# tlk00/BitMagic

Hardware: AMD Instinct MI355X
Metric: Gbits/s + % HBM roofline, 256-way fused AND+COUNT on 1B-bit vectors (higher is better)
Workload: dtype u64; 1 GPU; aggregator pipeline combine_and_sub counts-only: 256-way AND+COUNT, 256 x 1000000000-bit vectors in total, data set A (common 10% OR noise 10%: no early exit); vectors=256, bits_per_vector=1000000000, density_q16=6554, blocks_per_vector=15259, blocks_per_rank=15259, hbm_resident_bytes=32279432448

## Files before the change

### bitmagic_amd/csrc/bmx.hip

```cpp
#include "bmx_internal.h"
#ifdef BMX_DIAG
#include "bmx_diag.h"
#endif
#include "bmx_kernels2.h"
#include "bmx_kernels3.h"
#include "bmx_kernels4.h"
#include "bmx_kernels5.h"
#include "bmx_kernels6.h"
#include "bmx_kernels7.h"
#include "bmx_kernels8.h"
#include "bmx_kernels9.h"
#include "bmx_kernels10.h"
#include "bmx_kernels11.h"
#include "bmx_kernels12.h"
#include "bmx_kernels13.h"
#include "bmx_kernels14.h"

#include <algorithm>
#include <atomic>
#include <chrono>
#include <cstdio>
#include <cstdlib>
#include <cstring>
#include <new>
// ... 616 lines not shown
    }
    size_t need = (bytes + 63u) & ~(size_t)63u;
    if (ctx->stage_off + need > STAGE_BYTES) { HIPCHK(hipEventSynchronize(ctx->ev_stage)); ctx->stage_off = 0; }
    char* s = ctx->h_stage + ctx->stage_off;
    memcpy(s, src, bytes);
    ctx->stage_off += need;
    HIPCHK(hipMemcpyAsync(dst, s, bytes, hipMemcpyHostToDevice, ctx->stream));
    HIPCHK(hipEventRecord(ctx->ev_stage, ctx->stream));
    return BMX_OK;
}

static int coll_members_upload(bmx_ctx* ctx, const std::vector<u32>& ma, const std::vector<u32>& ms, DevBuf& d_buf, const u32** d_midx, const CollGroup** d_groups)
{
    const size_t nm = ma.size() + ms.size(), goff = (nm * 4 + 15) & ~(size_t)15;
    std::vector<u8> h(goff + sizeof(CollGroup));
    if (!ma.empty()) memcpy(h.data(), ma.data(), ma.size() * 4);
    if (!ms.empty()) memcpy(h.data() + ma.size() * 4, ms.data(), ms.size() * 4);
    const CollGroup g{0u, (u32)ma.size(), (u32)ma.size(), (u32)ms.size()};
    memcpy(h.data() + goff, &g, sizeof(g));
    int rc;
    if ((rc = dmalloc(ctx, &d_buf.p, h.size())) || (rc = h2d_staged(ctx, d_buf.p, h.data(), h.size()))) { d_buf.reset(); return rc; }
    *d_midx = (const u32*)d_buf.p; *d_groups = (const CollGroup*)((const char*)d_buf.p + goff);
    return BMX_OK;
}

static bool use_split(const bmx_ctx* ctx, const bmx_pipeline* p, u64 nitems)
{
    if (ctx->pipe_split == 0 || !nitems) return false;
    if (ctx->pipe_split == 1) return nitems <= 65535u * 16u;
    return nitems <= 384u && (u64)p->n_ops >= 24ull * p->ngroups;
}
#define SPLIT_WAVES 8

typedef void (*pipe_bits_fn)(const u64*, const u32*, const u32*, u32, u32, u32, u32, int, u64*);

static u32 pipe_window_cap(u32 wg)
{
    u32 wpb = wg / 64u;
    u32 per_cu = wpb >= 7u ? 1u : 12u / wpb;
    return 256u * per_cu * wpb;
}
static void pipe_plan(const bmx_ctx* ctx, u64 nitems, u32 ngroups, u32& rows, u32& wg, u32& unroll, u32& window)
{
    rows = (u32)ctx->pipe_rows;
    if (!rows) rows = nitems >= 1400u ? 8u : nitems >= 700u ? 4u : nitems >= 350u ? 2u : 1u;
    unroll = ctx->pipe_unroll ? (u32)ctx->pipe_unroll : ((rows >= 4u || !ctx->pipe_nt) ? 4u : 8u);
    u64 n = nitems * (8u / rows);
    wg = (u32)ctx->pipe_wg;
    if (!wg) {
        wg = 256u;
        if (rows == 8u) {
            static const u32 cand[3] = {640u, 768u, 512u};
            double best = -1.0;
            for (u32 c : cand) {
                u64 cap = pipe_window_cap(c), nwin = (n + cap - 1) / cap, per = (n + nwin - 1) / nwin;
                double fill = (double)per / (double)cap;
                if (fill > best + 0.02) { best = fill; wg = c; }
            }
        }
    }
    if (!ctx->pipe_nt && !ctx->pipe_wg && rows == 8u && wg > 512u) wg = 512u;
    if (ctx->pipe_window < 0 || (ctx->pipe_window == 0 && ngroups > 4u)) window = 0u;
    else if (ctx->pipe_window > 0) window = (u32)ctx->pipe_window;
    else window = (u32)std::max<u64>(pipe_window_cap(wg) / ((u64)ngroups * (8u / rows)), 1u);
}

template <int ROWS>
static pipe_bits_fn pipe_bits_rows(u32 unroll, bool nt, u32 wg)
// ... 21 lines not shown
            if (unroll == 4) return B2(4, true, 384);
            if constexpr (ROWS <= 4) { if (unroll == 8) return B2(8, true, 384); }
            if constexpr (ROWS <= 2) { if (unroll == 16) return B2(16, true, 384); }
        }
        if (nt && wg == 512 && unroll == 4) return B2(4, true, 512);
    }
#endif
#undef B2
    return nullptr;
}
static pipe_bits_fn pipe_bits_kernel(u32 rows, u32 unroll, bool nt, u32 wg)
{
    switch (rows) {
    case 8: return pipe_bits_rows<8>(unroll, nt, wg);
    case 4: return pipe_bits_rows<4>(unroll, nt, wg);
    case 2: return pipe_bits_rows<2>(unroll, nt, wg);
    case 1: return pipe_bits_rows<1>(unroll, nt, wg);
    default: return nullptr;
    }
}

static int ctx_set_tuning(bmx_ctx* ctx, const char* key, int value)
{
    ARGCHK(ctx && key);
    std::string k(key);
    if (k == "pipe_unroll") { ARGCHK(value == 0 || value == 1 || value == 2 || value == 4 || value == 8 || value == 16); ctx->pipe_unroll = value; }
    else if (k == "pipe_rows") { ARGCHK(value == 0 || value == 8 || value == 4 || value == 2 || value == 1); ctx->pipe_rows = value; }
    else if (k == "pipe_nt") ctx->pipe_nt = value != 0;
    else if (k == "pipe_lds") { ARGCHK(value >= 0 && value <= 160 * 1024); ctx->pipe_lds = value; }
    else if (k == "pipe_slots") { ARGCHK(value == 8 || value == 16); ctx->pipe_slots = value; }
    else if (k == "pipe_staged") { ARGCHK(value >= -1 && value <= 1); ctx->pipe_staged = value; }
    else if (k == "pipe_split") { ARGCHK(value >= -1 && value <= 1); ctx->pipe_split = value; }
    else if (k == "pipe_window") { ARGCHK(value >= -1); ctx->pipe_window = value; }
    else if (k == "or_tile") { ARGCHK(value >= 0 && value <= 3); ctx->or_tile = value; }
    else if (k == "or_rows") { ARGCHK(value >= -1 && value <= 1); ctx->or_rows = value; }
    else if (k == "or_depth") { ARGCHK(value == 4 || value == 8); ctx->or_depth = value; }
    else if (k == "direct_cols") { ARGCHK(value >= 0); ctx->direct_cols = value; }
    else if (k == "pair_stream") { ARGCHK(value == -1 || value == 0 || value == 2 || value == 4 || value == 8); ctx->pair_stream = value; }
    else if (k == "pair_wgs") { ARGCHK(value >= 1 && value <= 8); ctx->pair_wgs = value; }
    else if (k == "range_halves") { ARGCHK(value == 0 || value == 1); ctx->range_halves = value; }
    else if (k == "gap_count") { ARGCHK(value >= -1 && value <= 1); ctx->gap_count = value; }
    else if (k == "agg_shape") { ARGCHK(value == 0 || value == 1); ctx->agg_shape = value; }
    else if (k == "and_rows") { ARGCHK(value >= -1 && value <= 1); ctx->and_rows = value; }
    else if (k == "and_rows_wg") { ARGCHK(value == 128 || value == 256 || value == 512); ctx->and_rows_wg = value; }
    else if (k == "and_rows_depth") { ARGCHK(value == 2 || value == 3 || value == 4 || value == 8); ctx->and_rows_depth = value; }
    else if (k == "and_rows_nt") ctx->and_rows_nt = value != 0;
    else if (k == "and_rows_ipw") { ARGCHK(value >= 0 && value <= 64); ctx->and_rows_ipw = value; }
    else if (k == "ff_window") { ARGCHK(value >= -1); ctx->ff_window = value; }
    else if (k == "or_window") { ARGCHK(value >= -9); ctx->or_window = value; }
    else if (k == "gap_pack") { ARGCHK(value >= -1 && value <= 1); ctx->gap_pack = value; }
    else if (k == "coll_members") { ARGCHK(value >= -1 && value <= 1); ctx->coll_members = value; ++ctx->coll_gen; }
    else if (k == "coll_shape") { ARGCHK(value >= 0 && value <= 5); ctx->coll_shape = value; }
    else if (k == "op2_nt") { ARGCHK(value >= 0 && value <= 3); ctx->op2_nt = value; }
    else if (k == "op2_loop") { ARGCHK(value >= -1 && value <= 8); ctx->op2_loop = value; }
    else if (k == "op2_wgs") { ARGCHK(value >= 1 && value <= 8); ctx->op2_wgs = value; }
    else if (k == "pair_nt") { ARGCHK(value >= 0 && value <= 1); ctx->pair_nt = value; }
    else if (k == "pair_loop") { ARGCHK(value >= -1 && value <= 5); ctx->pair_loop = value; }
    else if (k == "eq_big_shape") { ARGCHK(value >= 0 && value <= 2); ctx->eq_big_shape = value; }
    else if (k == "eq_big") { ARGCHK(value >= -1 && value <= 1); ctx->eq_big = value; }
    else if (k == "coll_split") { ARGCHK(value == 0 || value == 1); ctx->coll_split = value; }
    else if (k == "coll_build") { ARGCHK(value >= -1 && value <= 1); ctx->coll_build = value; }
    else if (k == "coll_window") { ARGCHK(value >= 0); ctx->coll_window = value; }
    else if (k == "rs_select_lines") { ARGCHK(value >= 0 && value <= 2); ctx->rs_select_lines = value; }
    else if (k == "rs_sdir_shift") { ARGCHK(value == 0 || (value >= 6 && value <= 20)); ctx->rs_sdir_shift = value; }
    else if (k == "rs_lines") { ARGCHK(value >= 0 && value <= 2); ctx->rs_lines = value; }
    else if (k == "rs_sorted_hint") { ARGCHK(value == 0 || value == 1); ctx->rs_sorted_hint = value; }
// ... 112 lines not shown
    HIPCHK(hipGetDeviceCount(&n));
    if (device < 0 || device >= n) { g_last_error = "device index out of range"; return BMX_ERR_RANGE; }
    HIPCHK(hipSetDevice(device));
    Owned<bmx_ctx> ctx(new bmx_ctx());
    ctx->device = device;
    if (stream) ctx->stream = (hipStream_t)stream;
    else { HIPCHK(hipStreamCreateWithFlags(&ctx->stream, hipStreamNonBlocking)); ctx->own_stream = true; }
    HIPCHK(hipEventCreate(&ctx->ev0));
    HIPCHK(hipEventCreate(&ctx->ev1));
    HIPCHK(hipMalloc((void**)&ctx->d_small, 64 * sizeof(u64)));
    HIPCHK(hipHostMalloc((void**)&ctx->h_small, 64 * sizeof(u64)));
    HIPCHK(hipHostMalloc((void**)&ctx->h_stage, STAGE_BYTES));
    HIPCHK(hipEventCreateWithFlags(&ctx->ev_stage, hipEventDisableTiming));
    HIPCHK(hipMalloc((void**)&ctx->d_slots, COUNT_SLOTS * COUNT_SLOT_STRIDE * sizeof(u64)));
    HIPCHK(hipMemsetAsync(ctx->d_slots, 0, COUNT_SLOTS * COUNT_SLOT_STRIDE * sizeof(u64), ctx->stream));
    HIPCHK(hipMalloc((void**)&ctx->d_zero, 256));
    HIPCHK(hipMemsetAsync(ctx->d_zero, 0, 256, ctx->stream));
    HIPCHK(hipMalloc((void**)&ctx->d_done, FOLD_DONE_WORDS * 4));
    HIPCHK(hipMemsetAsync(ctx->d_done, 0, FOLD_DONE_WORDS * 4, ctx->stream));
    HIPCHK(hipMalloc((void**)&ctx->d_slots2, COUNT_SLOTS * COUNT_SLOT_STRIDE * sizeof(u64)));
    HIPCHK(hipMemsetAsync(ctx->d_slots2, 0, COUNT_SLOTS * COUNT_SLOT_STRIDE * sizeof(u64), ctx->stream));
    HIPCHK(hipMalloc((void**)&ctx->d_done2, FOLD_DONE_WORDS * 4));
    HIPCHK(hipMemsetAsync(ctx->d_done2, 0, FOLD_DONE_WORDS * 4, ctx->stream));
    HIPCHK(hipHostMalloc((void**)&ctx->h_pend, PEND_SLOTS * 8 * sizeof(u64)));
    HIPCHK(hipMalloc((void**)&ctx->d_cursor, 64));
    HIPCHK(hipMemsetAsync(ctx->d_cursor, 0, 64, ctx->stream));
    { int v = 0; if (hipDeviceGetAttribute(&v, hipDeviceAttributeMaxSharedMemoryPerBlock, device) == hipSuccess && v > 0) ctx->max_lds_bytes = (uint32_t)v; else (void)hipGetLastError(); }
    { size_t fr = 0, tot = 0; if (hipMemGetInfo(&fr, &tot) == hipSuccess && fr) ctx->pack_cap = (uint64_t)fr / 4; else (void)hipGetLastError(); }
    if (const char* e = getenv("BMX_DEBUG_REDZONE")) ctx->redzone = atoi(e) != 0;
    if (const char* e = getenv("BMX_PACK_MAX_MB")) { long long mb = atoll(e); if (mb >= 0) ctx->pack_cap = (uint64_t)mb << 20; }
    if (const char* e = getenv("BMX_POOL_MAX_MB")) { long long mb = atoll(e); if (mb >= 0) ctx->pool_cap = (uint64_t)mb << 20; }
    static const char* const env_keys[][2] = {
        {"BMX_PIPE_UNROLL", "pipe_unroll"}, {"BMX_PIPE_ROWS", "pipe_rows"}, {"BMX_PIPE_NT", "pipe_nt"},
        {"BMX_PIPE_WG", "pipe_wg"}, {"BMX_PIPE_WINDOW", "pipe_window"}, {"BMX_PIPE_SPLIT", "pipe_split"}, {"BMX_OR_TILE", "or_tile"}, {"BMX_OR_ROWS", "or_rows"}, {"BMX_OR_DEPTH", "or_depth"}, {"BMX_OR_WINDOW", "or_window"}, {"BMX_DIRECT_COLS", "direct_cols"}, {"BMX_FF_WINDOW", "ff_window"}, {"BMX_GAP_COUNT", "gap_count"}, {"BMX_AND_ROWS", "and_rows"}, {"BMX_AGG_SHAPE", "agg_shape"}, {"BMX_AND_ROWS_WG", "and_rows_wg"}, {"BMX_AND_ROWS_DEPTH", "and_rows_depth"}, {"BMX_AND_ROWS_NT", "and_rows_nt"}, {"BMX_AND_ROWS_IPW", "and_rows_ipw"}, {"BMX_RANGE_HALVES", "range_halves"}, {"BMX_PAIR_STREAM", "pair_stream"}, {"BMX_PAIR_WGS", "pair_wgs"}, {"BMX_RS_LANES", "rs_lanes"}, {"BMX_RS_SELECT_TOP", "rs_select_top"}, {"BMX_RS_SELECT_SEL", "rs_select_sel"}, {"BMX_RS_LINES", "rs_lines"}, {"BMX_RS_SELECT_LINES", "rs_select_lines"}, {"BMX_RS_SDIR_SHIFT", "rs_sdir_shift"}, {"BMX_COLL_SHAPE", "coll_shape"}, {"BMX_COLL_WINDOW", "coll_window"}, {"BMX_COLL_SPLIT", "coll_split"}, {"BMX_COLL_BUILD", "coll_build"}, {"BMX_EQ_BIG", "eq_big"}, {"BMX_PAIR_LOOP", "pair_loop"}, {"BMX_PAIR_NT", "pair_nt"}, {"BMX_EQ_BIG_SHAPE", "eq_big_shape"}, {"BMX_OP2_WGS", "op2_wgs"}, {"BMX_OP2_LOOP", "op2_loop"}, {"BMX_OP2_NT", "op2_nt"}, {"BMX_GAP_PACK", "gap_pack"}, {"BMX_COLL_MEMBERS", "coll_members"}, {"BMX_XCD_SWIZZLE", "xcd_swizzle"}};
    for (auto& kv : env_keys)
        if (const char* e = getenv(kv[0])) (void)ctx_set_tuning(ctx.get(), kv[1], atoi(e));
    g_last_error.clear();
    *out = ctx.release();
    return BMX_OK;
ABI_END }

int bmx_ctx_destroy(bmx_ctx* ctx) { ABI_TRY if (ctx) ctx_release(ctx); return BMX_OK; ABI_END }

int bmx_ctx_set_tuning(bmx_ctx* ctx, const char* key, int value) { ABI_TRY return ctx_set_tuning(ctx, key, value); ABI_END }

int bmx_probe_stream_rw(bmx_ctx* ctx, uint64_t bytes, int sets, int wgs_per_cu, int iters, float* ms_per_pass)
{ ABI_TRY
    ARGCHK(ctx && ms_per_pass && bytes >= 8192 && sets >= 1 && sets <= 8 && wgs_per_cu >= 1 && wgs_per_cu <= 8 && iters >= 1);
    int rc = set_dev(ctx); if (rc) return rc;
    const u64 nblk = bytes / 8192;
    if (nblk > 0x7FFFFFFFull) { g_last_error = "probe buffer too large"; return BMX_ERR_RANGE; }
    void* buf = nullptr;
    HIPCHK(hipMalloc(&buf, (size_t)nblk * 8192 * 3 * sets));
    hipError_t e = hipMemsetAsync(buf, 0x5A, (size_t)nblk * 8192 * 3 * sets, ctx->stream);
    const u32 waves = 4u, total = 256u * waves * (u32)wgs_per_cu;
    const u32 per_wave = (u32)((nblk + total - 1u) / total);
    const u32 grid = (u32)(((nblk + per_wave - 1u) / per_wave + waves - 1u) / waves);
    for (int it = -2; it < iters && e == hipSuccess; ++it) {
        if (it == 0) e = hipEventRecord(ctx->ev0, ctx->stream);
        uint4* base = (uint4*)buf + (size_t)((it + 2) % sets) * nblk * 512u * 3u;
        hipLaunchKernelGGL(HIP_KERNEL_NAME(k_probe_rw<4>), dim3(grid), dim3(256), 0, ctx->stream, (const uint4*)base, (const uint4*)(base + nblk * 512u),
                           base + 2u * nblk * 512u, (u32)nblk, per_wave);
    }
    if (e == hipSuccess) e = hipEventRecord(ctx->ev1, ctx->stream);
    if (e == hipSuccess) e = hipEventSynchronize(ctx->ev1);
    float ms = 0;
    if (e == hipSuccess) e = hipEventElapsedTime(&ms, ctx->ev0, ctx->ev1);
// ... 1150 lines not shown
                               (const u64* const*)p->d_udesc, (const u32*)p->d_unblk, p->nplanes, gv ? gv->gmask : (const u32*)p->d_gmask, gv ? gv->gskip : (const u32*)p->d_gskip, \
                               ngroups, nb_from, nb_to - nb_from, ctx->xcd_swz, (u64*)d_counts); } while (0)
            if (ctx->pipe_slots == 8) LAUNCH_STG(8); else LAUNCH_STG(16);
#undef LAUNCH_STG
            KCHK();
            return BMX_OK;
        }
    }
    if (use_split(ctx, p, nitems64)) {
        size_t lds = (size_t)SPLIT_WAVES * 8192;
        auto fn = k_pipe_split<2, SPLIT_WAVES>;
        HIPCHK(hipFuncSetAttribute(reinterpret_cast<const void*>(fn), hipFuncAttributeMaxDynamicSharedMemorySize, (int)lds));
        hipLaunchKernelGGL(fn, dim3((u32)nitems64), dim3(SPLIT_WAVES * 64), lds, ctx->stream,
                           (const u64*)p->d_dmat, row_off, and_n, sub_n, p->col_stride, ngroups, nb_from, nb_to, 0, (u64*)d_counts,
                           0, (uint4*)nullptr, (u64*)nullptr, (BlockStat*)nullptr);
        KCHK();
        return BMX_OK;
    }
    if (!p->has_gap) {
        u32 rows, wg, unroll, window;
        pipe_plan(ctx, nitems64, ngroups, rows, wg, unroll, window);
        u32 parts = 8u / rows;
        if (nitems64 * parts > 0xFFFFFFF0ull) { g_last_error = "too many work items in one run"; return BMX_ERR_RANGE; }
        pipe_bits_fn fn = pipe_bits_kernel(rows, unroll, ctx->pipe_nt != 0, wg);
        if (!fn) { g_last_error = "this (pipe_rows, pipe_unroll, pipe_nt, pipe_wg) shape is not compiled into the library"; return BMX_ERR_BADARG; }
        u32 wpb = wg / 64u;
        u32 ncols = nb_to - nb_from;
        u32 nwin = window ? (ncols + window - 1u) / window : 1u;
        u32 per = (ncols + nwin - 1u) / nwin;
        for (u32 c0 = 0; c0 < ncols; c0 += per) {
            u32 cols = std::min(per, ncols - c0);
            u32 nitems = cols * ngroups * parts, grid = (nitems + wpb - 1) / wpb;
            hipLaunchKernelGGL(fn, dim3(grid), dim3(wg), (size_t)ctx->pipe_lds, ctx->stream,
                               (const u64*)p->d_dmat, row_off, and_n, p->col_stride, ngroups, nb_from + c0, nitems, ctx->xcd_swz, (u64*)d_counts);
            KCHK();
        }
        return BMX_OK;
    }
    if (nitems64 > 0xFFFFFFF0ull) { g_last_error = "too many (column, group) items in one run"; return BMX_ERR_RANGE; }
    if (use_and_rows(ctx, p)) {
        const u32 ipw = ctx->and_rows_ipw > 0 ? (u32)ctx->and_rows_ipw : 1u;
        hipLaunchKernelGGL(and_rows_kernel<AR_COUNT>(ctx), dim3((u32)((nitems64 + ipw - 1u) / ipw)), dim3((u32)ctx->and_rows_wg), 0, ctx->stream,
                           (const u64*)p->d_dmat, row_off, and_n, sub_n, p->col_stride, ngroups, nb_from, (u32)nitems64, ctx->xcd_swz, (u64*)d_counts,
                           (uint4*)nullptr, (u64*)nullptr, (BlockStat*)nullptr, 0u, 0xFFFFFFFFu, and_rows_diag_bits(), ipw);
        KCHK();
        return BMX_OK;
    }
    if (use_gapcount(ctx, p)) {
        size_t lds = (size_t)(16384 * 2 + 2048) * 4;
        HIPCHK(hipFuncSetAttribute(reinterpret_cast<const void*>(k_pipe_counts_gapcount<false>), hipFuncAttributeMaxDynamicSharedMemorySize, (int)lds));
        hipLaunchKernelGGL(HIP_KERNEL_NAME(k_pipe_counts_gapcount<false>), dim3((u32)nitems64), dim3(1024), lds, ctx->stream,
                           p->d_dmat, row_off, and_n, sub_n, p->col_stride, ngroups, nb_from, (u32)nitems64, (u64*)d_counts,
                           (uint4*)nullptr, (u64*)nullptr, (BlockStat*)nullptr, 0u, 0xFFFFFFFFu);
        KCHK();
        return BMX_OK;
    }
    size_t lds = 4 * 2048 * 4;
    u32 ncols = nb_to - nb_from;
    u32 window = ctx->pipe_window > 0 ? (u32)ctx->pipe_window : 0u;
    u32 nwin = window ? (ncols + window - 1u) / window : 1u;
    u32 per = (ncols + nwin - 1u) / nwin;
    for (u32 c0 = 0; c0 < ncols; c0 += per) {
        u32 cols = std::min(per, ncols - c0);
        u32 nitems = cols * ngroups;
        u32 grid = (nitems + 3) / 4;
#define LAUNCH_PIPE(U) hipLaunchKernelGGL(HIP_KERNEL_NAME(k_pipe_counts<U>), dim3(grid), dim3(256), lds, ctx->stream, \
        p->d_dmat, row_off, and_n, sub_n, p->col_stride, ngroups, nb_from + c0, nitems, ctx->xcd_swz, (u64*)d_counts)
        switch (ctx->pipe_unroll) {
        case 1: LAUNCH_PIPE(1); break;
        case 2: LAUNCH_PIPE(2); break;
        default: LAUNCH_PIPE(4); break;
        }
#undef LAUNCH_PIPE
        KCHK();
    }
    return BMX_OK;
}

int bmx_pipeline_describe(bmx_ctx* ctx, bmx_pipeline* p, uint32_t nb_from, uint32_t nb_to, char* buf, size_t buf_len, uint32_t* n_launches)
{ ABI_TRY
    ARGCHK(ctx && p && p->ctx == ctx && buf && buf_len > 0);
    if (n_launches) *n_launches = 1;
    int rc = pipe_range(p, nb_from, nb_to); if (rc) return rc;
    u64 nitems64 = (u64)(nb_to - nb_from) * p->ngroups;
    bool reuse = p->ngroups >= 32 && (uint64_t)p->n_ops >= 8ull * p->nplanes;
    if (!p->h_uids.empty() && ctx->gap_pack != 0 && p->cm_gen == ctx->coll_gen && coll_by_id(ctx, p->cm_a_id) && (!p->cm_s_id || coll_by_id(ctx, p->cm_s_id))) {
        if (p->cm_full) snprintf(buf, buf_len, "k_coll_apply<AND_COUNT,512> x 1 launch, %llu workgroups (packed collection of the operand set)", (unsigned long long)nitems64);
        else snprintf(buf, buf_len, "k_coll_members<AND_COUNT> x 1 launch, a wave per (column, group): %u x %u items (members of a packed collection)", nb_to - nb_from, p->ngroups);
    }
    else if (p->staged_ok && (ctx->pipe_staged == 1 || (ctx->pipe_staged < 0 && reuse)))
        snprintf(buf, buf_len, "k_pipe_counts_staged<%d> x 1 launch, %u workgroups", ctx->pipe_slots, nb_to - nb_from);
    else if (use_split(ctx, p, nitems64))
        snprintf(buf, buf_len, "k_pipe_split<2,%d> x 1 launch, %llu workgroups", SPLIT_WAVES, (unsigned long long)nitems64);
    else if (use_and_rows(ctx, p))
        snprintf(buf, buf_len, "k_agg_and_rows<COUNT,%d,%d> x 1 launch, %llu workgroups", ctx->and_rows_wg, ctx->and_rows_depth, (unsigned long long)nitems64);
    else if (use_gapcount(ctx, p))
        snprintf(buf, buf_len, "k_pipe_counts_gapcount x 1 launch, %llu workgroups", (unsigned long long)nitems64);
    else if (p->has_gap)
        snprintf(buf, buf_len, "k_pipe_counts<%d> x 1 launch", ctx->pipe_unroll == 1 ? 1 : ctx->pipe_unroll == 2 ? 2 : 4);
    else {
// ... 1970 lines not shown
```

### bitmagic_amd/csrc/bmx_device.h

```cpp
#pragma once
#include <hip/hip_runtime.h>
#include <stdint.h>

typedef uint8_t  u8;
typedef uint16_t u16;
typedef uint32_t u32;
typedef uint64_t u64;

#define GMETA(e) ((u32)((e) >> 48) & 0x1FFFu)
#define GMETA_NONE 0xFFFFFFFFu
#define BMX_DESC_KIND(d) ((u32)((d) & 3ull))
#define BMX_DESC_PTR(d)  ((d) & ~3ull)

typedef u32 u32x4 __attribute__((ext_vector_type(4)));
typedef const __attribute__((address_space(1))) u32x4* gcptr4;
typedef __attribute__((address_space(1))) u32x4* gptr4;
typedef const __attribute__((address_space(1))) u16* gcptr16;

template <int ROWS> struct Part { u32x4 r[ROWS]; };
typedef Part<8> Blk;

__device__ __forceinline__ gcptr4 as_gc4(u64 addr) { return (gcptr4)(uintptr_t)addr; }
__device__ __forceinline__ gcptr4 as_gc4(const void* p) { return (gcptr4)(uintptr_t)p; }
__device__ __forceinline__ gptr4 as_g4(void* p) { return (gptr4)(uintptr_t)p; }
// ... 640 lines not shown
        bool one = (s ^ ((k - 1u) & 1u)) != 0u;
        c += one ? ((k == 1u) ? e + 1u : e - pe) : 0u;
    }
    return c;
}

__device__ __forceinline__ u64 mix64(u64 x)
{
    x ^= x >> 30; x *= 0xBF58476D1CE4E5B9ull;
    x ^= x >> 27; x *= 0x94D049BB133111EBull;
    x ^= x >> 31;
    return x;
}
__device__ __forceinline__ u64 gen_word64(u64 seed, u32 vec_id, u64 w64, u32 d)
{
    if (d >= 65536u) return ~0ull;
    u64 base = seed ^ ((u64)vec_id * 0x9E3779B97F4A7C15ull);
    u64 acc = 0;
#pragma unroll
    for (u32 k = 0; k < 16; ++k) {
        u64 r = mix64(base + (w64 * 16u + k) * 0xD6E8FEB86659FD93ull);
        acc = ((d >> k) & 1u) ? (acc | r) : (acc & r);
    }
    return acc;
}

__device__ __forceinline__ u64 readlane64(u64 v, u32 l)
{
    u32 lo = __builtin_amdgcn_readlane((u32)v, l);
    u32 hi = __builtin_amdgcn_readlane((u32)(v >> 32), l);
    return ((u64)hi << 32) | lo;
}

template <int U, bool NT, int OPK, int ROWS = 8>
__device__ __forceinline__ bool pipe_chain(Part<ROWS>& acc, const u64* __restrict__ plist, u32 n, u32 lane, u32 poff = 0u)
{
    if (n == 0) return false;
    u64 pn[U];
    auto fetch = [&](u32 k) {
#pragma unroll
        for (int u = 0; u < U; ++u) pn[u] = plist[k + u < n ? k + u : n - 1u];
    };
    auto issue = [&](Part<ROWS>* buf) {
#pragma unroll
        for (int u = 0; u < U; ++u) part_load<ROWS, NT>(buf[u], as_gc4(uniform64(pn[u])) + poff, lane);
    };
    auto consume = [&](Part<ROWS>* buf) {
#pragma unroll
        for (int u = 0; u < U; ++u)
#pragma unroll
            for (int i = 0; i < ROWS; ++i) {
                if constexpr (OPK == 0) acc.r[i] &= buf[u].r[i];
                else if constexpr (OPK == 1) acc.r[i] &= ~buf[u].r[i];
                else acc.r[i] |= buf[u].r[i];
            }
        if constexpr (OPK == 2) return part_is_ones<ROWS>(acc); else return part_is_zero<ROWS>(acc);
    };
    Part<ROWS> A[U], B[U];
    u32 k = U;
    fetch(0);
    issue(A);
    fetch(k);
    bool zero;
    do {
        issue(B); fetch(k + U);
        bool z1 = consume(A);
        issue(A); fetch(k + 2 * U);
        bool z2 = consume(B);
        zero = z1 | z2;
        k += 2 * U;
    } while (!zero && k < n + U);
    return zero;
}
```

### bitmagic_amd/csrc/bmx_internal.h

```cpp
#pragma once
#include "../../include/bmx.h"
#include <hip/hip_runtime.h>
#include <stdint.h>

#include <map>
#include <memory>
#include <string>
#include <unordered_map>
#include <vector>

typedef uint8_t  u8;
typedef uint16_t u16;
typedef uint32_t u32;
typedef uint64_t u64;

int bmx_fail_hip(hipError_t e, const char* what, const char* file, int line);
void bmx_set_last_error(const char* msg);
#define HIPCHK(call) do { hipError_t e_ = (call); if (e_ != hipSuccess) return bmx_fail_hip(e_, #call, __FILE__, __LINE__); } while (0)
#define ARGCHK(cond) do { if (!(cond)) { bmx_set_last_error("bad argument: " #cond); return BMX_ERR_BADARG; } } while (0)
#define KCHK() HIPCHK(hipGetLastError())
#define PEND_SLOTS 1024
#include <new>
#include <stdexcept>
int bmx_abi_caught(int kind, const char* what);
// ... 6 lines not shown

struct bmx_ctx {
    int device = 0;
    hipStream_t stream = nullptr;
    bool own_stream = false;
    hipEvent_t ev0 = nullptr, ev1 = nullptr;
    uint64_t mem_used = 0;
    void* scratch = nullptr; size_t scratch_bytes = 0;
    void* aux = nullptr; size_t aux_bytes = 0;
    u64* d_small = nullptr;
    u64* d_slots = nullptr;
    u64* d_slots2 = nullptr; u32* d_done2 = nullptr;
    u64* h_pend = nullptr; uint64_t pend_used[16] = {};
    u64* d_cursor = nullptr;
    u64* d_zero = nullptr;
    u32* d_done = nullptr;
    u64* h_small = nullptr;
    char* h_stage = nullptr; size_t stage_off = 0;
    hipEvent_t ev_stage = nullptr;
    std::multimap<size_t, void*> pool_free;
    std::unordered_map<void*, size_t> pool_live;
    uint64_t pool_cached = 0, pool_cap = 16ull << 30;
    struct RzInfo { void* raw; size_t block; size_t bytes; int line; };
    bool redzone = false;
    std::unordered_map<void*, RzInfo> rz_live;
    uint64_t rz_hits = 0; std::string rz_report;
    long long fail_dmalloc_after = -1;
    bool fail_dmalloc_throws = false;
    int pipe_unroll = 0;
    int pipe_rows = 0;
    int pipe_nt = 1;
    int pipe_wg = 0;
    int pipe_window = 0;
    int pipe_staged = -1;
    int pipe_lds = 0;
    int pipe_slots = 16;
    int pipe_split = -1;
    int or_tile = 0;
    int direct_cols = 384;
    int pair_stream = -1;
    int pair_wgs = 1;
    int range_halves = 1;
    int gap_count = -1;
    int agg_shape = 0;
    int and_rows = -1;
    int and_rows_wg = 256;
    int and_rows_ipw = 0;
    int and_rows_nt = 0;
    int and_rows_depth = 3;
    int ff_window = 0;
    int or_window = 0;
    int or_rows = -1;
    int or_depth = 4;
    std::vector<struct bmx_coll*> colls;
    int gap_pack = -1;
    uint64_t pack_cap = 16ull << 30, pack_bytes = 0, coll_tick = 0;
    uint64_t coll_gen = 0, coll_next_id = 0;
    int coll_members = -1;
    int coll_building = 0;
    std::unordered_map<uint64_t, struct bmx_vec*> live_vecs;
    float last_pack_ms = 0.f;
    uint32_t max_lds_bytes = 160u * 1024u;
    int coll_split = 1;
    int coll_build = -1;
    int coll_shape = 4;
    int pair_nt = 1;
// ... 119 lines not shown
```

### bitmagic_amd/csrc/bmx_kernels.h

```cpp
#pragma once
#include "bmx_device.h"

#define DESC_MAKE(ptr, kind) ((u64)(uintptr_t)(ptr) | ((u64)(kind) << 62))
#define DESC_K(d) ((u32)((d) >> 62))
#define DESC_P(d) ((d) & 0x0000FFFFFFFFFFFFull)
#define DESC_MAKE_GAP(ptr, len, sbit) (DESC_MAKE(ptr, K_GAP) | ((u64)((((u32)(len)) << 1) | ((u32)(sbit) & 1u)) << 48))
enum { K_NULL = 0, K_FULL = 1, K_BIT = 2, K_GAP = 3 };

#define ROW_EMPTY 1ull
#define ROW_FULL  2ull
#define ROW_ONES  4ull

struct BlockStat { u32 pop; u32 runs; u32 first; u32 kind; };

__global__ __launch_bounds__(256)
void k_generate(u64 seed, u32 vec_id, int with_common, u32 d, u64 nbits, u64* __restrict__ out, u64 nwords64, u64 word0)
{
    u64 i = (u64)blockIdx.x * blockDim.x + threadIdx.x;
    u64 stride = (u64)gridDim.x * blockDim.x;
    for (; i < nwords64; i += stride) {
        u64 w = word0 + i;
        u64 v = gen_word64(seed, vec_id, w, d);
        if (with_common) v |= gen_word64(seed, 0xFFFFFFFFu, w, d);
        u64 bit0 = w * 64u;
// ... 330 lines not shown
{
    u32 lane = lane_id();
    u64 wid = (u64)blockIdx.x * (blockDim.x >> 6) + (threadIdx.x >> 6);
    if (wid >= (u64)ncols * ngroups) return;
    u32 c = (u32)(wid / ngroups), g = (u32)(wid - (u64)c * ngroups);
    u64* row = dmat + (size_t)c * col_stride + po.row_off[g];
    u32 na = po.and_n[g], ns = po.sub_n[g];
    u32 ao = po.and_off[g], so = po.sub_off[g];
    u32 nbit = 0, ngap = 0, sbit = 0, sgap = 0;
    bool empty = (na == 0);
    if (na && sort_operands(po.desc, po.nblocks, ao, na, c, K_NULL, row + 2, nbit, ngap, lane)) empty = true;
    if (!empty && ns && sort_operands(po.desc, po.nblocks, so, ns, c, K_FULL, row + 2 + na, sbit, sgap, lane)) empty = true;
    u64 flags = 0;
    if (empty) flags = ROW_EMPTY;
    else if (!nbit && !ngap) { if (!sbit && !sgap) flags = ROW_FULL; else flags = ROW_ONES; }
    else if (!nbit) flags = ROW_ONES;
    if (lane == 0) {
        row[0] = (u64)nbit | ((u64)ngap << 16) | ((u64)sbit << 32) | ((u64)sgap << 48);
        row[1] = flags;
    }
}

__device__ __forceinline__ u32 xcd_remap(u32 b, u32 nwg)
{
    u32 q = nwg >> 3, rem = nwg & 7u;
    u32 x = b & 7u, i = b >> 3;
    return x * q + (x < rem ? x : rem) + i;
}

template <int U>
__global__ __launch_bounds__(256)
void k_pipe_counts(const u64* __restrict__ dmat, const u32* __restrict__ row_off,
                   const u32* __restrict__ and_n, const u32* __restrict__ sub_n, u32 col_stride,
                   u32 ngroups, u32 col_from, u32 nitems, int xcd_swz, u64* __restrict__ counts)
{
    extern __shared__ u32 lds_dyn[];
    u32 lane = lane_id(), wave = threadIdx.x >> 6;
    u32 bid = xcd_swz ? xcd_remap(blockIdx.x, gridDim.x) : blockIdx.x;
    u32 item = uniform32(bid * 4u + wave);
    if (item >= nitems) return;
    u32 c = item / ngroups, g = item - c * ngroups;
    const u64* row = dmat + (size_t)(col_from + c) * col_stride + row_off[g];
    u64 hdr = uniform64(row[0]), flags = uniform64(row[1]);
    if (flags & ROW_EMPTY) return;
    if (flags & ROW_FULL) { if (lane == 0) atomicAdd(reinterpret_cast<unsigned long long*>(&counts[g]), 65536ull); return; }
    u32 nba = (u32)(hdr & 0xFFFFu), nga = (u32)((hdr >> 16) & 0xFFFFu);
    u32 nbs = (u32)((hdr >> 32) & 0xFFFFu), ngs = (u32)(hdr >> 48);
    u32 na = uniform32(and_n[g]), ns = uniform32(sub_n[g]);
    const u64* pa = row + 2;
    const u64* ps = pa + na;
    u32* lds = lds_dyn + wave * 2048u;

    Blk acc;
    blk_fill(acc, ~0u);
    if (pipe_chain<U, true, 0>(acc, pa, nba, lane)) return;
    if (pipe_chain<U, true, 1>(acc, ps, nbs, lane)) return;
    if (nga | ngs) {
        blk_to_lds(acc, lds, lane);
        if (nga && gap_apply_list<GAP_AND>(pa + na - 1u, nga, lds, lane)) return;
        if (ngs && gap_apply_list<GAP_SUB>(ps + ns - 1u, ngs, lds, lane)) return;
        blk_from_lds(acc, lds, lane);
    }
    u32 cnt = wave_sum(blk_lane_popcount(acc));
    if (lane == 0 && cnt) atomicAdd(reinterpret_cast<unsigned long long*>(&counts[g]), (unsigned long long)cnt);
}

template <int U, bool NT, int WG = 256, int ROWS = 8>
__global__ __launch_bounds__(WG)
void k_pipe_counts_bits2(const u64* __restrict__ dmat, const u32* __restrict__ row_off,
                         const u32* __restrict__ and_n, u32 col_stride,
                         u32 ngroups, u32 col_from, u32 nitems, int xcd_swz, u64* __restrict__ counts)
{
    constexpr u32 PARTS = 8 / ROWS;
    u32 lane = lane_id(), wave = threadIdx.x >> 6, wpb = blockDim.x >> 6;
    u32 bid = xcd_swz ? xcd_remap(blockIdx.x, gridDim.x) : blockIdx.x;
    u32 item = uniform32(bid * wpb + wave);
    if (item >= nitems) return;
    u32 part = item % PARTS, cg = item / PARTS;
    u32 c = cg / ngroups, g = cg - c * ngroups;
    const u64* row = dmat + (size_t)(col_from + c) * col_stride + row_off[g];
    u64 hdr = uniform64(row[0]), flags = uniform64(row[1]);
    if (flags & ROW_EMPTY) return;
    if (flags & ROW_FULL) { if (lane == 0) atomicAdd(reinterpret_cast<unsigned long long*>(&counts[g]), (unsigned long long)(65536u / PARTS)); return; }
    u32 nba = (u32)(hdr & 0xFFFFu), nbs = (u32)((hdr >> 32) & 0xFFFFu);
    u32 na = uniform32(and_n[g]);
    const u64* pa = row + 2;
    const u64* ps = pa + na;
    const u32 poff = part * ROWS * 64u;
    Part<ROWS> acc;
#pragma unroll
    for (int i = 0; i < ROWS; ++i) acc.r[i] = (u32x4)(~0u);
    if (pipe_chain<U, NT, 0, ROWS>(acc, pa, nba, lane, poff)) return;
    if (pipe_chain<U, NT, 1, ROWS>(acc, ps, nbs, lane, poff)) return;
    u32 cnt = 0;
#pragma unroll
    for (int i = 0; i < ROWS; ++i) {
        cnt += __popcll(((u64)acc.r[i].y << 32) | acc.r[i].x);
        cnt += __popcll(((u64)acc.r[i].w << 32) | acc.r[i].z);
    }
    cnt = wave_sum(cnt);
    if (lane == 0 && cnt) atomicAdd(reinterpret_cast<unsigned long long*>(&counts[g]), (unsigned long long)cnt);
}

#ifdef BMX_DIAG
template <int AUX>
__global__ __launch_bounds__(256)
void k_diag_stream_read_buf(const uint4* __restrict__ buf, u64 nblocks8k, u32 blocks_per_wave, int pattern, int xcd_swz, u64* __restrict__ sink)
{
    u32 lane = lane_id();
    u32 bid = xcd_swz ? xcd_remap(blockIdx.x, gridDim.x) : blockIdx.x;
    u64 w = (u64)bid * (blockDim.x >> 6) + (threadIdx.x >> 6);
    u64 nwaves = nblocks8k / blocks_per_wave;
    if (w >= nwaves) return;
    u64 b0 = pattern ? w : w * blocks_per_wave;
    u64 step = pattern ? nwaves : 1;
    u32x4 acc = (u32x4)(0u);
    for (u32 j = 0; j < blocks_per_wave; ++j) {
        u64 addr = uniform64((u64)(uintptr_t)(buf + (b0 + j * step) * 512u));
        __amdgpu_buffer_rsrc_t r = __builtin_amdgcn_make_buffer_rsrc((void*)(uintptr_t)addr, 0, 8192, 0x00020000);
#pragma unroll
        for (int i = 0; i < 8; ++i) acc |= __builtin_amdgcn_raw_buffer_load_b128(r, (int)(i * 1024 + lane * 16), 0, AUX);
    }
    if ((acc.x | acc.y | acc.z | acc.w) == 0x12345678u) sink[0] = 1;
}

#endif
// ... 50 lines not shown
```

Before: 55710 Gbit/s.

## Switch AND chain to narrow per-row fold once few lanes remain live

The pipelined AND/AND-NOT chain now tracks how many lanes still hold nonzero accumulator bits. Once that count drops to a threshold (default 16), it switches to a narrow fold that walks only the still-nonzero rows per lane and loads just those segments. Lanes drop out as their segments become zero. This is meant to avoid streaming full blocks from HBM when most of the block is already zero. The cost is an extra ballot and popcount per step, a serialized per-row loop with divergence, and less memory-level parallelism in the narrow phase.

```diff
diff --git a/bitmagic_amd/csrc/bmx.hip b/bitmagic_amd/csrc/bmx.hip
--- a/bitmagic_amd/csrc/bmx.hip
+++ b/bitmagic_amd/csrc/bmx.hip
@@ -672,8 +672,10 @@
 }
 #define SPLIT_WAVES 8
 
-typedef void (*pipe_bits_fn)(const u64*, const u32*, const u32*, u32, u32, u32, u32, int, u64*);
-
+typedef void (*pipe_bits_fn)(const u64*, const u32*, const u32*, u32, u32, u32, u32, int, u64*, u32);
+
+static const u32 PIPE_NARROW_DEFAULT = 16u;
+static u32 pipe_narrow_t(const bmx_ctx* ctx) { return ctx->pipe_narrow < 0 ? PIPE_NARROW_DEFAULT : (u32)ctx->pipe_narrow; }
 static u32 pipe_window_cap(u32 wg)
 {
     u32 wpb = wg / 64u;
@@ -761,6 +763,7 @@
     else if (k == "pipe_staged") { ARGCHK(value >= -1 && value <= 1); ctx->pipe_staged = value; }
     else if (k == "pipe_split") { ARGCHK(value >= -1 && value <= 1); ctx->pipe_split = value; }
     else if (k == "pipe_window") { ARGCHK(value >= -1); ctx->pipe_window = value; }
+    else if (k == "pipe_narrow") { ARGCHK(value >= -1 && value <= 64); ctx->pipe_narrow = value; }
     else if (k == "or_tile") { ARGCHK(value >= 0 && value <= 3); ctx->or_tile = value; }
     else if (k == "or_rows") { ARGCHK(value >= -1 && value <= 1); ctx->or_rows = value; }
     else if (k == "or_depth") { ARGCHK(value == 4 || value == 8); ctx->or_depth = value; }
@@ -939,7 +942,7 @@
     if (const char* e = getenv("BMX_POOL_MAX_MB")) { long long mb = atoll(e); if (mb >= 0) ctx->pool_cap = (uint64_t)mb << 20; }
     static const char* const env_keys[][2] = {
         {"BMX_PIPE_UNROLL", "pipe_unroll"}, {"BMX_PIPE_ROWS", "pipe_rows"}, {"BMX_PIPE_NT", "pipe_nt"},
-        {"BMX_PIPE_WG", "pipe_wg"}, {"BMX_PIPE_WINDOW", "pipe_window"}, {"BMX_PIPE_SPLIT", "pipe_split"}, {"BMX_OR_TILE", "or_tile"}, {"BMX_OR_ROWS", "or_rows"}, {"BMX_OR_DEPTH", "or_depth"}, {"BMX_OR_WINDOW", "or_window"}, {"BMX_DIRECT_COLS", "direct_cols"}, {"BMX_FF_WINDOW", "ff_window"}, {"BMX_GAP_COUNT", "gap_count"}, {"BMX_AND_ROWS", "and_rows"}, {"BMX_AGG_SHAPE", "agg_shape"}, {"BMX_AND_ROWS_WG", "and_rows_wg"}, {"BMX_AND_ROWS_DEPTH", "and_rows_depth"}, {"BMX_AND_ROWS_NT", "and_rows_nt"}, {"BMX_AND_ROWS_IPW", "and_rows_ipw"}, {"BMX_RANGE_HALVES", "range_halves"}, {"BMX_PAIR_STREAM", "pair_stream"}, {"BMX_PAIR_WGS", "pair_wgs"}, {"BMX_RS_LANES", "rs_lanes"}, {"BMX_RS_SELECT_TOP", "rs_select_top"}, {"BMX_RS_SELECT_SEL", "rs_select_sel"}, {"BMX_RS_LINES", "rs_lines"}, {"BMX_RS_SELECT_LINES", "rs_select_lines"}, {"BMX_RS_SDIR_SHIFT", "rs_sdir_shift"}, {"BMX_COLL_SHAPE", "coll_shape"}, {"BMX_COLL_WINDOW", "coll_window"}, {"BMX_COLL_SPLIT", "coll_split"}, {"BMX_COLL_BUILD", "coll_build"}, {"BMX_EQ_BIG", "eq_big"}, {"BMX_PAIR_LOOP", "pair_loop"}, {"BMX_PAIR_NT", "pair_nt"}, {"BMX_EQ_BIG_SHAPE", "eq_big_shape"}, {"BMX_OP2_WGS", "op2_wgs"}, {"BMX_OP2_LOOP", "op2_loop"}, {"BMX_OP2_NT", "op2_nt"}, {"BMX_GAP_PACK", "gap_pack"}, {"BMX_COLL_MEMBERS", "coll_members"}, {"BMX_XCD_SWIZZLE", "xcd_swizzle"}};
+        {"BMX_PIPE_WG", "pipe_wg"}, {"BMX_PIPE_WINDOW", "pipe_window"}, {"BMX_PIPE_NARROW", "pipe_narrow"},{"BMX_PIPE_SPLIT", "pipe_split"}, {"BMX_OR_TILE", "or_tile"}, {"BMX_OR_ROWS", "or_rows"}, {"BMX_OR_DEPTH", "or_depth"}, {"BMX_OR_WINDOW", "or_window"}, {"BMX_DIRECT_COLS", "direct_cols"}, {"BMX_FF_WINDOW", "ff_window"}, {"BMX_GAP_COUNT", "gap_count"}, {"BMX_AND_ROWS", "and_rows"}, {"BMX_AGG_SHAPE", "agg_shape"}, {"BMX_AND_ROWS_WG", "and_rows_wg"}, {"BMX_AND_ROWS_DEPTH", "and_rows_depth"}, {"BMX_AND_ROWS_NT", "and_rows_nt"}, {"BMX_AND_ROWS_IPW", "and_rows_ipw"}, {"BMX_RANGE_HALVES", "range_halves"}, {"BMX_PAIR_STREAM", "pair_stream"}, {"BMX_PAIR_WGS", "pair_wgs"}, {"BMX_RS_LANES", "rs_lanes"}, {"BMX_RS_SELECT_TOP", "rs_select_top"}, {"BMX_RS_SELECT_SEL", "rs_select_sel"}, {"BMX_RS_LINES", "rs_lines"}, {"BMX_RS_SELECT_LINES", "rs_select_lines"}, {"BMX_RS_SDIR_SHIFT", "rs_sdir_shift"}, {"BMX_COLL_SHAPE", "coll_shape"}, {"BMX_COLL_WINDOW", "coll_window"}, {"BMX_COLL_SPLIT", "coll_split"}, {"BMX_COLL_BUILD", "coll_build"}, {"BMX_EQ_BIG", "eq_big"}, {"BMX_PAIR_LOOP", "pair_loop"}, {"BMX_PAIR_NT", "pair_nt"}, {"BMX_EQ_BIG_SHAPE", "eq_big_shape"}, {"BMX_OP2_WGS", "op2_wgs"}, {"BMX_OP2_LOOP", "op2_loop"}, {"BMX_OP2_NT", "op2_nt"}, {"BMX_GAP_PACK", "gap_pack"}, {"BMX_COLL_MEMBERS", "coll_members"}, {"BMX_XCD_SWIZZLE", "xcd_swizzle"}};
     for (auto& kv : env_keys)
         if (const char* e = getenv(kv[0])) (void)ctx_set_tuning(ctx.get(), kv[1], atoi(e));
     g_last_error.clear();
@@ -2156,7 +2159,7 @@
             u32 cols = std::min(per, ncols - c0);
             u32 nitems = cols * ngroups * parts, grid = (nitems + wpb - 1) / wpb;
             hipLaunchKernelGGL(fn, dim3(grid), dim3(wg), (size_t)ctx->pipe_lds, ctx->stream,
-                               (const u64*)p->d_dmat, row_off, and_n, p->col_stride, ngroups, nb_from + c0, nitems, ctx->xcd_swz, (u64*)d_counts);
+                               (const u64*)p->d_dmat, row_off, and_n, p->col_stride, ngroups, nb_from + c0, nitems, ctx->xcd_swz, (u64*)d_counts, pipe_narrow_t(ctx));
             KCHK();
         }
         return BMX_OK;
@@ -2189,7 +2192,7 @@
         u32 nitems = cols * ngroups;
         u32 grid = (nitems + 3) / 4;
 #define LAUNCH_PIPE(U) hipLaunchKernelGGL(HIP_KERNEL_NAME(k_pipe_counts<U>), dim3(grid), dim3(256), lds, ctx->stream, \
-        p->d_dmat, row_off, and_n, sub_n, p->col_stride, ngroups, nb_from + c0, nitems, ctx->xcd_swz, (u64*)d_counts)
+        p->d_dmat, row_off, and_n, sub_n, p->col_stride, ngroups, nb_from + c0, nitems, ctx->xcd_swz, (u64*)d_counts, pipe_narrow_t(ctx))
         switch (ctx->pipe_unroll) {
         case 1: LAUNCH_PIPE(1); break;
         case 2: LAUNCH_PIPE(2); break;
diff --git a/bitmagic_amd/csrc/bmx_device.h b/bitmagic_amd/csrc/bmx_device.h
--- a/bitmagic_amd/csrc/bmx_device.h
+++ b/bitmagic_amd/csrc/bmx_device.h
@@ -696,8 +696,63 @@
     return ((u64)hi << 32) | lo;
 }
 
-template <int U, bool NT, int OPK, int ROWS = 8>
-__device__ __forceinline__ bool pipe_chain(Part<ROWS>& acc, const u64* __restrict__ plist, u32 n, u32 lane, u32 poff = 0u)
+template <int ROWS>
+__device__ __forceinline__ u32 part_live_lanes(const Part<ROWS>& b)
+{
+    u32 v = 0;
+#pragma unroll
+    for (int i = 0; i < ROWS; ++i) v |= b.r[i].x | b.r[i].y | b.r[i].z | b.r[i].w;
+    return (u32)__popcll(__ballot(v != 0u));
+}
+
+#define PIPE_NARROW_DEPTH 16
+template <bool NT, int OPK, int ROWS>
+__device__ __forceinline__ bool pipe_narrow_fold(Part<ROWS>& acc, const u64* __restrict__ plist, u32 k0, u32 n, u32 lane, u32 poff)
+{
+    static_assert(OPK == 0 || OPK == 1, "narrow fold: AND / AND-NOT only");
+    u32 m = 0;
+#pragma unroll
+    for (int i = 0; i < ROWS; ++i) m |= ((acc.r[i].x | acc.r[i].y | acc.r[i].z | acc.r[i].w) != 0u) ? (1u << i) : 0u;
+    bool left = false;
+    while (__ballot(m != 0u) != 0ull) {
+        const bool mine = m != 0u;
+        const u32 rp = mine ? (u32)__builtin_ctz(m) : 0u;
+        m &= m - 1u;
+        u32x4 cacc = (u32x4)(0u);
+#pragma unroll
+        for (int i = 0; i < ROWS; ++i) cacc = (mine && rp == (u32)i) ? acc.r[i] : cacc;
+        const u32 off = poff + rp * 64u + lane;
+        bool on = mine;
+        for (u32 k = k0; k < n; k += PIPE_NARROW_DEPTH) {
+            u64 pk[PIPE_NARROW_DEPTH];
+#pragma unroll
+            for (int u = 0; u < PIPE_NARROW_DEPTH; ++u) pk[u] = plist[k + u < n ? k + u : n - 1u];
+            if (on) {
+                u32x4 x[PIPE_NARROW_DEPTH];
+#pragma unroll
+                for (int u = 0; u < PIPE_NARROW_DEPTH; ++u) {
+                    gcptr4 q = as_gc4(uniform64(pk[u])) + off;
+                    if constexpr (NT) x[u] = __builtin_nontemporal_load(q); else x[u] = *q;
+                }
+#pragma unroll
+                for (int u = 0; u < PIPE_NARROW_DEPTH; ++u) { if constexpr (OPK == 0) cacc &= x[u]; else cacc &= ~x[u]; }
+                on = (cacc.x | cacc.y | cacc.z | cacc.w) != 0u;
+            }
+            if (__ballot(on) == 0ull) break;
+        }
+#pragma unroll
+        for (int i = 0; i < ROWS; ++i) acc.r[i] = (mine && rp == (u32)i) ? cacc : acc.r[i];
+        left |= on;
+    }
+    return __ballot(left) == 0ull;
+}
+
+#ifndef BMX_PIPE_PEEL
+#define BMX_PIPE_PEEL 1
+#endif
+
+template <int U, bool NT, int OPK, int ROWS = 8, bool NARROW = false>
+__device__ __forceinline__ bool pipe_chain(Part<ROWS>& acc, const u64* __restrict__ plist, u32 n, u32 lane, u32 poff = 0u, u32 narrow_t = 0u)
 {
     if (n == 0) return false;
     u64 pn[U];
@@ -720,19 +775,53 @@
             }
         if constexpr (OPK == 2) return part_is_ones<ROWS>(acc); else return part_is_zero<ROWS>(acc);
     };
-    Part<ROWS> A[U], B[U];
-    u32 k = U;
-    fetch(0);
-    issue(A);
-    fetch(k);
-    bool zero;
-    do {
-        issue(B); fetch(k + U);
-        bool z1 = consume(A);
-        issue(A); fetch(k + 2 * U);
-        bool z2 = consume(B);
-        zero = z1 | z2;
-        k += 2 * U;
-    } while (!zero && k < n + U);
-    return zero;
-}
+    if constexpr (!NARROW || OPK == 2) {
+        Part<ROWS> A[U], B[U];
+        u32 k = U;
+        fetch(0);
+        issue(A);
+        fetch(k);
+        bool zero;
+        do {
+            issue(B); fetch(k + U);
+            bool z1 = consume(A);
+            issue(A); fetch(k + 2 * U);
+            bool z2 = consume(B);
+            zero = z1 | z2;
+            k += 2 * U;
+        } while (!zero && k < n + U);
+        return zero;
+    } else {
+        auto live_after = [&](Part<ROWS>* buf) { (void)consume(buf); return part_live_lanes<ROWS>(acc); };
+        u32 kn = 0;
+        if (part_live_lanes<ROWS>(acc) > narrow_t) {
+            Part<ROWS> A[U], B[U];
+            fetch(0);
+            issue(A);
+            fetch(U);
+#if BMX_PIPE_PEEL == 1
+            issue(B); fetch(2 * U);
+#endif
+            u32 live = live_after(A);
+            kn = U;
+            if (live > narrow_t && n > U) {
+#if BMX_PIPE_PEEL != 1
+                issue(B); fetch(2 * U);
+#endif
+                u32 k = 2 * U;
+                u32 l1;
+                do {
+                    issue(A); fetch(k + U);
+                    l1 = live_after(B);
+                    issue(B); fetch(k + 2 * U);
+                    live = live_after(A);
+                    k += 2 * U;
+                } while (l1 != 0u && live > narrow_t && k < n + U);
+                kn = k - U;
+            }
+            if (live == 0u) return true;
+            if (kn >= n) return false;
+        }
+        return pipe_narrow_fold<NT, OPK, ROWS>(acc, plist, kn, n, lane, poff);
+    }
+}
diff --git a/bitmagic_amd/csrc/bmx_internal.h b/bitmagic_amd/csrc/bmx_internal.h
--- a/bitmagic_amd/csrc/bmx_internal.h
+++ b/bitmagic_amd/csrc/bmx_internal.h
@@ -62,6 +62,7 @@
     int pipe_nt = 1;
     int pipe_wg = 0;
     int pipe_window = 0;
+    int pipe_narrow = -1;
     int pipe_staged = -1;
     int pipe_lds = 0;
     int pipe_slots = 16;
diff --git a/bitmagic_amd/csrc/bmx_kernels.h b/bitmagic_amd/csrc/bmx_kernels.h
--- a/bitmagic_amd/csrc/bmx_kernels.h
+++ b/bitmagic_amd/csrc/bmx_kernels.h
@@ -386,7 +386,7 @@
 __global__ __launch_bounds__(256)
 void k_pipe_counts(const u64* __restrict__ dmat, const u32* __restrict__ row_off,
                    const u32* __restrict__ and_n, const u32* __restrict__ sub_n, u32 col_stride,
-                   u32 ngroups, u32 col_from, u32 nitems, int xcd_swz, u64* __restrict__ counts)
+                   u32 ngroups, u32 col_from, u32 nitems, int xcd_swz, u64* __restrict__ counts, u32 narrow_t)
 {
     extern __shared__ u32 lds_dyn[];
     u32 lane = lane_id(), wave = threadIdx.x >> 6;
@@ -407,8 +407,8 @@
 
     Blk acc;
     blk_fill(acc, ~0u);
-    if (pipe_chain<U, true, 0>(acc, pa, nba, lane)) return;
-    if (pipe_chain<U, true, 1>(acc, ps, nbs, lane)) return;
+    if (pipe_chain<U, true, 0, 8, true>(acc, pa, nba, lane, 0u, narrow_t)) return;
+    if (pipe_chain<U, true, 1, 8, true>(acc, ps, nbs, lane, 0u, narrow_t)) return;
     if (nga | ngs) {
         blk_to_lds(acc, lds, lane);
         if (nga && gap_apply_list<GAP_AND>(pa + na - 1u, nga, lds, lane)) return;
@@ -423,7 +423,7 @@
 __global__ __launch_bounds__(WG)
 void k_pipe_counts_bits2(const u64* __restrict__ dmat, const u32* __restrict__ row_off,
                          const u32* __restrict__ and_n, u32 col_stride,
-                         u32 ngroups, u32 col_from, u32 nitems, int xcd_swz, u64* __restrict__ counts)
+                         u32 ngroups, u32 col_from, u32 nitems, int xcd_swz, u64* __restrict__ counts, u32 narrow_t)
 {
     constexpr u32 PARTS = 8 / ROWS;
     u32 lane = lane_id(), wave = threadIdx.x >> 6, wpb = blockDim.x >> 6;
@@ -444,8 +444,8 @@
     Part<ROWS> acc;
 #pragma unroll
     for (int i = 0; i < ROWS; ++i) acc.r[i] = (u32x4)(~0u);
-    if (pipe_chain<U, NT, 0, ROWS>(acc, pa, nba, lane, poff)) return;
-    if (pipe_chain<U, NT, 1, ROWS>(acc, ps, nbs, lane, poff)) return;
+    if (pipe_chain<U, NT, 0, ROWS, true>(acc, pa, nba, lane, poff, narrow_t)) return;
+    if (pipe_chain<U, NT, 1, ROWS, true>(acc, ps, nbs, lane, poff, narrow_t)) return;
     u32 cnt = 0;
 #pragma unroll
     for (int i = 0; i < ROWS; ++i) {
```

After: 54270 Gbit/s. -2.6%, worse.
